# ViktorLiang/GW-Depth

Measured on AMD Instinct MI355X. Metric: images/sec (train fwd+bwd) 480x640 bs=8/GPU, higher is better.
Workload: dtype bf16; 1 GPU; GW-Depth full model (res50 + DETR 6+6 + 4-scale ReferTransformer + decoder) fwd+17 losses+bwd+clip+AdamW, 480x640, bs=8/GPU, dropout 0.1; global_batch=8, parallelism=dp1, launch=hipgraph, graph_segments=1, grad_buckets=8

## Files before the change

### gw_depth_amd/hip.py

```python
import ctypes
import os

import torch

_HERE = os.path.dirname(os.path.abspath(__file__))
LIB_PATH = os.environ.get("GWD_LIB") or os.path.join(_HERE, "libgwdepth_hip.so")

F32, BF16 = 0, 1
ACT_NONE, ACT_RELU, ACT_GELU, ACT_ELU, ACT_SIGMOID = 0, 1, 2, 3, 4
WS_INORM_GELU, WS_RESAMPLE_BWD, WS_EVAL, WS_PLANE, WS_HEALTH, WS_REGIONS, WS_FUSION = 0, 1, 2, 3, 4, 5, 6
GATHER_CONV, GATHER_TRANSPOSED, GATHER_UPSAMPLED = 0, 1, 2
RESAMPLE_BILINEAR_AC, RESAMPLE_NEAREST = 0, 1

ENTRY_POINTS = [
    "gwd_version", "gwd_arch", "gwd_conv_forward", "gwd_conv_wgrad", "gwd_weight_prep", "gwd_act_backward",
    "gwd_colsum", "gwd_layernorm_forward", "gwd_layernorm_backward", "gwd_softmax_forward",
    "gwd_softmax_backward", "gwd_silog_sums", "gwd_silog_backward", "gwd_seg_ce_sum", "gwd_seg_ce_backward",
    "gwd_sqnorm", "gwd_adamw_step", "gwd_resample_forward", "gwd_resample_backward", "gwd_avgpool_forward",
    "gwd_avgpool_backward", "gwd_winattn_forward", "gwd_winattn_backward", "gwd_tokattn_forward",
    "gwd_tokattn_backward", "gwd_tokattn_pair_forward", "gwd_tokattn_pair_backward", "gwd_upsample_taps_collapse", "gwd_upsample_taps_fold", "gwd_certain_sample", "gwd_lsap", "gwd_window_map", "gwd_window_map_multi",
    "gwd_inorm_gelu_forward", "gwd_inorm_gelu_backward", "gwd_weight_prep_batch",
    "gwd_point_sample_forward", "gwd_point_sample_backward", "gwd_act_backward_colsum", "gwd_resample_backward_sep",
    "gwd_softmax_masked_forward", "gwd_softmax_scaled_backward", "gwd_query_workspace", "gwd_eval_accumulate", "gwd_colsum_batch", "gwd_conv_wgrad_batch",
    "gwd_conv_wgrad_takes_bias",
    "gwd_plane_loss_forward", "gwd_plane_loss_backward", "gwd_collate",
    "gwd_anchor_depth_forward", "gwd_anchor_depth_backward", "gwd_mha_flash_forward", "gwd_mha_flash_backward",
    "gwd_ref_scores_forward", "gwd_ref_scores_backward", "gwd_ref_mix_forward", "gwd_ref_mix_backward", "gwd_unpad_add_batch", "gwd_stem_pack", "gwd_stem_forward", "gwd_pos_sine", "gwd_silog_finalize", "gwd_psp_pool_forward", "gwd_psp_pool_backward",
    "gwd_match_cost", "gwd_set_losses_forward", "gwd_set_losses_backward", "gwd_set_losses_focal_forward", "gwd_set_losses_focal_backward", "gwd_resample_u8_pass", "gwd_gather2d", "gwd_point_sample_backward_gather", "gwd_point_sample_framed_forward", "gwd_point_sample_framed_backward", "gwd_stride_place", "gwd_color_adjust", "gwd_bmm",
    "gwd_dense_postprocess", "gwd_line_postprocess", "gwd_line_score",
    "gwd_dense_postprocess_resized",
    "gwd_resample_u8_pass_batch", "gwd_gather2d_batch", "gwd_color_adjust_batch",
    "gwd_pyr_tail_forward", "gwd_pyr_tail_backward", "gwd_pyr_tail_fold_wgrad",
    "gwd_widen_u16_batch",
    "gwd_line_nms",
    "gwd_eval_frames",
    "gwd_segment_stats", "gwd_health_decide", "gwd_adamw_step_guarded",
    "gwd_adamw_step_ema", "gwd_ema_swap",
    "gwd_glass_regions", "gwd_region_planes", "gwd_depth_planar",
    "gwd_line_profiles",
    "gwd_fusion_ring", "gwd_fusion_planes", "gwd_fusion_depth",
    "gwd_render_frames",
]


class HipUnavailable(RuntimeError):
    pass


class ConvDesc(ctypes.Structure):
    _fields_ = [("x", ctypes.c_void_p), ("w", ctypes.c_void_p), ("y", ctypes.c_void_p), ("z", ctypes.c_void_p),
                ("scale", ctypes.c_void_p), ("shift", ctypes.c_void_p), ("residual", ctypes.c_void_p),
                ("zero_page", ctypes.c_void_p), ("mult", ctypes.c_void_p), ("gate", ctypes.c_void_p)] + \
               [(n, ctypes.c_int32) for n in ("B", "Hi", "Wi", "Cin", "Ho", "Wo", "Cout", "KH", "KW", "stride", "pad",
                                              "gather", "Hv", "Wv", "act")] + \
               [("act_scale", ctypes.c_float), ("dtype", ctypes.c_int32), ("gate_act", ctypes.c_int32),
                ("ln_mean", ctypes.c_void_p), ("ln_rstd", ctypes.c_void_p), ("ln_C", ctypes.c_int32), ("reserved", ctypes.c_int32),
                ("dbias", ctypes.c_void_p)]


class BmmDesc(ctypes.Structure):
    _fields_ = [("a", ctypes.c_void_p), ("b", ctypes.c_void_p), ("c", ctypes.c_void_p)] + \
               [(n, ctypes.c_int64) for n in ("a_sb0", "a_sb1", "a_ld", "b_sb0", "b_sb1", "b_ld", "c_sb0", "c_sb1", "c_ld")] + \
               [(n, ctypes.c_int32) for n in ("M", "N", "K", "nb0", "nb1", "a_kmajor", "b_kmajor", "c_is_f32_accumulate", "splits")] + \
               [("alpha", ctypes.c_float), ("dtype", ctypes.c_int32)]


class PrepJob(ctypes.Structure):
    _fields_ = [("w", ctypes.c_void_p), ("row_scale", ctypes.c_void_p), ("w_fwd", ctypes.c_void_p), ("w_dgrad", ctypes.c_void_p),
                ("N", ctypes.c_int32), ("taps", ctypes.c_int32), ("C", ctypes.c_int32), ("block0", ctypes.c_int32),
                ("Np", ctypes.c_int32), ("Cg", ctypes.c_int32), ("Cgp", ctypes.c_int32), ("reserved", ctypes.c_int32)]


class UnpadJob(ctypes.Structure):
    _fields_ = [("src", ctypes.c_void_p), ("dst", ctypes.c_void_p), ("N", ctypes.c_int32), ("taps", ctypes.c_int32), ("G", ctypes.c_int32),
                ("Cg", ctypes.c_int32), ("Cgp", ctypes.c_int32), ("block0", ctypes.c_int32)]


# ... 100 lines not shown


def _zero_page(device):
    if device.type != "cuda":
        return None
    z = _ZERO_PAGES.get(device)
    if z is None:
        z = _ZERO_PAGES[device] = torch.zeros(256, dtype=torch.uint8, device=device)
    return ctypes.c_void_p(z.data_ptr())


def dtype_code(t):
    if t.dtype == torch.float32:
        return F32
    if t.dtype == torch.bfloat16:
        return BF16
    raise TypeError("gw_depth_amd kernels take float32 or bfloat16, got %s" % t.dtype)


def _ptr_pitched(t):
    return None if t is None else ctypes.c_void_p(t.data_ptr())


def _ptr(t):
    if t is None:
        return None
    if not t.is_contiguous():
        raise ValueError("kernel operand must be contiguous")
    return ctypes.c_void_p(t.data_ptr())


class HipLibrary:

    def __init__(self, path=LIB_PATH):
        if not os.path.exists(path):
            raise HipUnavailable(
                "libgwdepth_hip.so not built (%s); run `python -c 'import __graft_entry__ as g; g.build()'`" % path)
        self.lib = ctypes.CDLL(path)
        for name in ENTRY_POINTS:
            if not hasattr(self.lib, name):
                raise HipUnavailable("libgwdepth_hip.so lacks symbol " + name)
        self.lib.gwd_arch.restype = ctypes.c_char_p
        for name in ENTRY_POINTS[2:]:
            getattr(self.lib, name).restype = ctypes.c_int
        L = self.lib
        vp, i32, i64, f32 = ctypes.c_void_p, ctypes.c_int32, ctypes.c_int64, ctypes.c_float
        L.gwd_conv_forward.argtypes = [ctypes.POINTER(ConvDesc), vp]
        L.gwd_conv_wgrad.argtypes = [ctypes.POINTER(ConvDesc), vp, vp]
        L.gwd_weight_prep.argtypes = [vp, vp, vp, vp, i32, i32, i32, i32, vp]
        L.gwd_act_backward.argtypes = [vp, vp, vp, vp, i64, i32, i32, f32, i32, vp]
        L.gwd_colsum.argtypes = [vp, vp, i64, i32, i32, vp]
        L.gwd_conv_wgrad_batch.argtypes = [ctypes.POINTER(ConvDesc), ctypes.POINTER(ctypes.c_void_p), i32, vp]
        L.gwd_conv_wgrad_takes_bias.argtypes = [ctypes.POINTER(ConvDesc), i32]
        L.gwd_plane_loss_forward.argtypes = [vp, vp, vp, vp, i32, i32, i32, i32, vp, vp, vp, i32, vp]
        L.gwd_plane_loss_backward.argtypes = [vp, vp, vp, vp, i32, i32, i32, vp, vp, vp, i32, vp]
        L.gwd_collate.argtypes = [ctypes.POINTER(ImageJob), i32, i32, i32, ctypes.POINTER(ctypes.c_float),
                                  ctypes.POINTER(ctypes.c_float), vp, vp, vp, vp, i32, vp]
        L.gwd_mha_flash_forward.argtypes = [vp, vp, vp, i64, i64, i64, vp, vp, vp, i64, vp, i32, i32, i32, i32, f32, i32, vp]
        L.gwd_mha_flash_backward.argtypes = [vp] * 5 + [i64] * 5 + [vp] * 7 + [i64] * 3 + [i32, i32, i32, i32, f32, i32, vp]
        L.gwd_anchor_depth_forward.argtypes = [vp, vp, vp, i32, i64, i32, i32, vp]
        L.gwd_anchor_depth_backward.argtypes = [vp, vp, vp, vp, vp, i32, i64, i32, i32, vp]
        L.gwd_colsum_batch.argtypes = [ctypes.POINTER(ColsumJob), i32, i32, vp]
        L.gwd_layernorm_forward.argtypes = [vp, vp, vp, vp, vp, vp, vp, i64, i32, i32, i32, i32, vp]
        L.gwd_layernorm_backward.argtypes = [vp, vp, vp, vp, vp, vp, vp, vp, vp, i64, i32, i32, i32, vp, i32, vp]
        L.gwd_unpad_add_batch.argtypes = [ctypes.POINTER(UnpadJob), i32, vp]
        L.gwd_silog_finalize.argtypes = [vp, f32, f32, vp, vp]
        L.gwd_resample_u8_pass.argtypes = [vp, vp, vp, vp, i32, i32, i32, i32, i32, i64, i32, i32, i32, i32, vp]
        L.gwd_gather2d.argtypes = [vp, vp, vp, vp, i32, i32, i64, i32, vp]
        L.gwd_resample_u8_pass_batch.argtypes = [ctypes.POINTER(ResampleJob), i32, i32, i32, vp, i64, vp]
        L.gwd_gather2d_batch.argtypes = [ctypes.POINTER(GatherJob), i32, vp, i64, vp]
        L.gwd_color_adjust_batch.argtypes = [ctypes.POINTER(ColorJob), i32, vp, i32, vp]
        L.gwd_match_cost.argtypes = [vp] * 5 + [i32] * 6 + [f32, f32, vp]
        L.gwd_set_losses_forward.argtypes = [vp] * 9 + [f32] + [vp] * 4 + [i32] * 6 + [vp]
        L.gwd_set_losses_backward.argtypes = [vp] * 8 + [f32] + [vp] * 6 + [i32] * 6 + [vp]
        L.gwd_set_losses_focal_forward.argtypes = [vp] * 9 + [f32] * 2 + [vp] * 4 + [i32] * 6 + [vp]
        L.gwd_set_losses_focal_backward.argtypes = [vp] * 8 + [f32] * 2 + [vp] * 6 + [i32] * 6 + [vp]
        L.gwd_color_adjust.argtypes = [vp, vp, vp, i64, i32, f32, vp]
        L.gwd_bmm.argtypes = [ctypes.POINTER(BmmDesc), vp]
        L.gwd_stride_place.argtypes = [vp, vp, vp] + [i32] * 8 + [vp]
        L.gwd_psp_pool_forward.argtypes = [vp] * 5 + [i32] * 5 + [vp]
        L.gwd_psp_pool_backward.argtypes = [vp] * 6 + [i32] * 6 + [vp]
        L.gwd_pos_sine.argtypes = [vp, vp, vp, vp, vp, i32, i32, i32, i32, i32, i32, i32, vp]
        L.gwd_stem_pack.argtypes = [vp, vp, vp, vp]
        L.gwd_stem_forward.argtypes = [vp, vp, vp, vp, i32, i32, i32, i32, vp]
        L.gwd_softmax_forward.argtypes = [vp, vp, i64, i32, i32, vp]
        L.gwd_softmax_backward.argtypes = [vp, vp, vp, i64, i32, i32, vp]
        L.gwd_silog_sums.argtypes = [vp, vp, vp, i32, i32, i32, i32, i32, i32, i32, vp]
        L.gwd_silog_backward.argtypes = [vp, vp, vp, vp, f32, f32, vp, i32, i32, i32, i32, i32, i32, i32, vp]
        L.gwd_seg_ce_sum.argtypes = [vp, vp, vp, i64, i32, vp]
        L.gwd_seg_ce_backward.argtypes = [vp, vp, vp, f32, vp, i64, i32, vp]
        L.gwd_resample_forward.argtypes = [vp, vp] + [i32] * 9 + [vp]
        L.gwd_resample_backward.argtypes = [vp, vp] + [i32] * 7 + [vp, i32, i32, vp]
        L.gwd_avgpool_forward.argtypes = [vp, vp] + [i32] * 6 + [vp]
        L.gwd_avgpool_backward.argtypes = [vp, vp] + [i32] * 6 + [vp]
        sp = ctypes.POINTER(Strided)
        L.gwd_winattn_forward.argtypes = [sp, sp, sp, sp, vp, vp, i32, vp, i64, i32, i32, i32, f32, i32, vp]
        L.gwd_winattn_backward.argtypes = [sp] * 7 + [vp, vp, vp, i32, vp, i64, i32, i32, i32, f32, i32, i32, vp]
        L.gwd_ref_scores_forward.argtypes = [sp, vp, vp, i32, i32, i32, i32, i32, f32, i32, vp]
        L.gwd_ref_scores_backward.argtypes = [sp, vp, vp, sp, vp, i32, i32, i32, i32, i32, f32, i32, vp]
        L.gwd_ref_mix_forward.argtypes = [vp, vp, vp, vp, i32, i32, i32, i32, i32, i32, vp]
        L.gwd_ref_mix_backward.argtypes = [vp, vp, vp, vp, vp, i32, i32, i32, i32, i32, i32, vp]
        L.gwd_tokattn_forward.argtypes = [sp] * 4 + [i64, i32, i32, f32, i32, vp]
        L.gwd_tokattn_backward.argtypes = [sp] * 7 + [i64, i32, i32, f32, i32, vp]
        L.gwd_upsample_taps_collapse.argtypes = [vp, vp, i32, i32, i32, vp]
        L.gwd_upsample_taps_fold.argtypes = [vp, vp, i32, i32, vp]
        L.gwd_tokattn_pair_forward.argtypes = [sp] * 6 + [i64, i32, i32, f32, i32, vp]
# ... 65 lines not shown
        if n < 0:
            raise ValueError("gwd_query_workspace(%d, %r) -> %d" % (op, dims, n))
        return n

    def version(self):
        return self.lib.gwd_version()

    @staticmethod
    def _desc(x, w, y, dims, z=None, scale=None, shift=None, residual=None, stride=1, pad=0,
              gather=GATHER_CONV, virt=(0, 0), act=ACT_NONE, act_scale=1.0, mult=None, gate=None, gate_act=ACT_NONE, ln=None,
              zero_page=True, dbias=None):
        B, Hi, Wi, Cin, Ho, Wo, Cout, KH, KW = dims
        d = ConvDesc()
        d.x, d.w, d.y, d.z = _ptr(x), _ptr(w), _ptr(y), _ptr(z)
        d.scale, d.shift, d.residual = _ptr(scale), _ptr(shift), _ptr(residual)
        d.zero_page = _zero_page(x.device) if zero_page else None
        d.mult = _ptr(mult)
        d.gate, d.gate_act = _ptr(gate), (gate_act if gate is not None else ACT_NONE)
        d.B, d.Hi, d.Wi, d.Cin, d.Ho, d.Wo, d.Cout, d.KH, d.KW = B, Hi, Wi, Cin, Ho, Wo, Cout, KH, KW
        d.stride, d.pad, d.gather, d.Hv, d.Wv = stride, pad, gather, virt[0], virt[1]
        d.act, d.act_scale, d.dtype = act, act_scale, dtype_code(x)
        if ln is not None:
            d.ln_mean, d.ln_rstd, d.ln_C = _ptr(ln[0]), _ptr(ln[1]), int(ln[2])
        d.dbias = _ptr(dbias)
        return d

    def conv_forward(self, x, w, y, dims, **kw):
        d = self._desc(x, w, y, dims, **kw)
        rc = self.lib.gwd_conv_forward(ctypes.byref(d), self._stream(x, w, y))
        if rc == -4 and kw.get("ln") is not None:
            return False
        if rc == -4 and kw.get("gate") is not None and kw.get("gate_act") == ACT_GELU:
            return False
        self._check(rc, "gwd_conv_forward")

    def conv_wgrad(self, x, gy, dw, dims, **kw):
        d = self._desc(x, None, gy, dims, **kw)
        self._check(self.lib.gwd_conv_wgrad(ctypes.byref(d), _ptr(dw), self._stream(x, gy, dw, kw.get("dbias"))), "gwd_conv_wgrad")

    def conv_wgrad_takes_bias(self, x, gy, dims, batched, **kw):
        d = self._desc(x, None, gy, dims, **kw)
        return self.lib.gwd_conv_wgrad_takes_bias(ctypes.byref(d), 1 if batched else 0) == 1

    def conv_wgrad_batch(self, jobs):
        descs = (ConvDesc * len(jobs))()
        dws = (ctypes.c_void_p * len(jobs))()
        ts = []
        for i, (x, gy, dw, dims, kw) in enumerate(jobs):
            descs[i] = self._desc(x, None, gy, dims, **kw)
            dws[i] = _ptr(dw)
            ts += [x, gy, dw, kw.get("dbias")]
        self._check(self.lib.gwd_conv_wgrad_batch(descs, dws, len(jobs), self._stream(*ts)), "gwd_conv_wgrad_batch")

    def weight_prep(self, w, row_scale, w_fwd, w_dgrad, N, taps, C, dtype):
        self._check(self.lib.gwd_weight_prep(_ptr(w), _ptr(row_scale), _ptr(w_fwd), _ptr(w_dgrad), N, taps, C, dtype,
                                             self._stream(w, w_fwd, w_dgrad)), "gwd_weight_prep")

    def act_backward(self, gy, ref, gx, scale, rows, C, act, act_scale):
        self._check(self.lib.gwd_act_backward(_ptr(gy), _ptr(ref), _ptr(gx), _ptr(scale), rows, C, act, act_scale,
                                              dtype_code(gy), self._stream(gy, ref, gx)), "gwd_act_backward")

    def act_backward_colsum(self, gy, ref, gx, dbias, rows, C, act, act_scale, mult=None):
        rc = self.lib.gwd_act_backward_colsum(_ptr(gy), _ptr(ref), _ptr(gx), _ptr(dbias), rows, C, act, act_scale, _ptr(mult),
                                              dtype_code(gy), self._stream(gy, ref, gx))
        if rc == -4:
            return False
        self._check(rc, "gwd_act_backward_colsum")
        return True

    def colsum(self, g, out, rows, C):
        self._check(self.lib.gwd_colsum(_ptr(g), _ptr(out), rows, C, dtype_code(g), self._stream(g, out)), "gwd_colsum")

    def colsum_batch(self, jobs):
        recs = (ColsumJob * len(jobs))()
        for r, (g, out, rows, C) in zip(recs, jobs):
            r.g, r.out, r.rows, r.C = g.data_ptr(), out.data_ptr(), rows, C
            if not (g.is_contiguous() and out.is_contiguous()):
                raise ValueError("kernel operand must be contiguous")
        ts = [t for j in jobs for t in j[:2]]
        self._check(self.lib.gwd_colsum_batch(recs, len(jobs), dtype_code(jobs[0][0]), self._stream(*ts)), "gwd_colsum_batch")

    @staticmethod
    def colsum_batchable(g, C):
        vec = 8 if g.dtype == torch.bfloat16 else 4
        return C % vec == 0 and C // vec <= 256

    def layernorm_forward(self, x, gamma, beta, y, mean, rstd, rows, C, gelu, residual=None, ld=0):
        self._check(self.lib.gwd_layernorm_forward(_ptr(x), _ptr(gamma), _ptr(beta), _ptr(residual), _ptr(y), _ptr(mean), _ptr(rstd),
                                                   rows, C, ld, int(gelu), dtype_code(x), self._stream(x, y)),
                    "gwd_layernorm_forward")

    def layernorm_backward(self, gy, x, gamma, beta, mean, rstd, gx, dgamma, dbeta, rows, C, gelu, ld=0, gskip=None, elu_input=False):
        flags = int(bool(gelu)) | (2 if elu_input else 0)
        rc = self.lib.gwd_layernorm_backward(_ptr(gy), _ptr(x), _ptr(gamma), _ptr(beta), _ptr(mean), _ptr(rstd), _ptr(gx), _ptr(dgamma),
                                             _ptr(dbeta), rows, C, ld, flags, _ptr(gskip), dtype_code(x), self._stream(gy, x, gx))
        if rc == -4 and (gskip is not None or elu_input):
            self._check(self.lib.gwd_layernorm_backward(_ptr(gy), _ptr(x), _ptr(gamma), _ptr(beta), _ptr(mean), _ptr(rstd), _ptr(gx), _ptr(dgamma),
                                                        _ptr(dbeta), rows, C, ld, int(bool(gelu)), None, dtype_code(x), self._stream(gy, x, gx)),
                        "gwd_layernorm_backward")
            return False
        self._check(rc, "gwd_layernorm_backward")
        return True

    def pos_counts(self, mask_full, mask_level, counts):
        B, H, W = mask_full.shape
        _, h, w = mask_level.shape
# ... 924 lines not shown
```

### gw_depth_amd/model.py

```python
import math
import os

import torch
import torch.nn.functional as F
from torch import nn

from . import ops
from .layers import Conv, FrozenBN, LayerNorm, Linear, Mlp, MlpNorm, Seq
from .ops import ACT_ELU, ACT_GELU, ACT_NONE, ACT_RELU, ACT_SIGMOID

WS = 7
HEADS = 16
DEFAULT_FP32_STAGES = ()


class NestedTensor:

    def __init__(self, tensors, mask):
        self.tensors, self.mask = tensors, mask

    def to(self, device):
        return NestedTensor(self.tensors.to(device), None if self.mask is None else self.mask.to(device))

    def decompose(self):
# ... 753 lines not shown
    def __init__(self, cin, cout):
        super().__init__()
        self.conv = Conv(cin, cout, 3)

    def forward(self, x, size, defer=False, in_gate=ACT_NONE):
        return ops.conv2d(x, self.conv.weight, pad=1, act=ACT_ELU, upsample_to=size, defer=defer, in_gate=in_gate)


class DensePrediction(nn.Module):

    def __init__(self, max_depth, tdim, feat=64):
        super().__init__()
        self.max_depth = max_depth
        self.depth_token_fuse = Mlp(feat + 1 + tdim, None, tdim)
        self.seg_token_fuse = Mlp(feat + tdim, None, tdim)
        for tag in ("depth", "seg"):
            setattr(self, f"upconv1_{tag}", UpConv(tdim, tdim))
            setattr(self, f"norm_{tag}", LayerNorm(tdim))
            setattr(self, f"conv1_{tag}", Seq(_0=Conv(tdim, tdim, 3)))
            setattr(self, f"upconv2_{tag}", UpConv(tdim, tdim // 2))
            setattr(self, f"conv2_{tag}", Seq(_0=Conv(tdim // 2, tdim // 2, 3)))
            if tag == "depth":
                self.get_depth = Seq(_0=Conv(tdim // 2, 1, 3))
        self.get_seg = Conv(tdim // 2, 2, 3)

    def fuse_padded(self, x):
        fc1, fc2 = self.depth_token_fuse.fc1, self.depth_token_fuse.fc2
        pad = x.shape[-1] - fc1.weight.shape[-1]
        if pad == 0:
            return self.depth_token_fuse(x)
        w1 = ops.derived_weight(fc1.weight, pad, lambda: F.pad(fc1.weight, (0, pad, 0, pad)))
        w2 = ops.derived_weight(fc2.weight, pad, lambda: F.pad(fc2.weight, (0, pad)))
        h = ops.linear(x, w1, F.pad(fc1.bias, (0, pad)), ACT_GELU)
        return ops.linear(h, w2, fc2.bias)

    _ZERO_BLOCKS = {}

    @classmethod
    def zero_channels(cls, like, n):
        key = (tuple(like.shape[:3]), n, like.dtype, str(like.device))
        z = cls._ZERO_BLOCKS.get(key)
        if z is None:
            z = cls._ZERO_BLOCKS[key] = torch.zeros(tuple(like.shape[:3]) + (n,), dtype=like.dtype, device=like.device)
        return z

    def branch(self, fuse_in, tag, fuse, size, cast):
        B, H, W, _ = fuse_in.shape
        f = fuse(cast("decoder_fuse", fuse_in))
        f = cast("decoder_up1", f)
        u1 = getattr(self, f"norm_{tag}")(getattr(self, f"upconv1_{tag}")(f, (2 * H, 2 * W), defer=True), in_gate=ACT_ELU)
        c1 = ops.conv2d(u1, getattr(self, f"conv1_{tag}")[0].weight, pad=1, act=ACT_ELU, defer=True)
        c1 = cast("decoder_up2", c1)
        u2 = getattr(self, f"upconv2_{tag}")(c1, size, defer=True, in_gate=ACT_ELU)
        return cast("decoder_head", ops.conv2d(u2, getattr(self, f"conv2_{tag}")[0].weight, pad=1, act=ACT_ELU, in_gate=ACT_ELU))

    def forward(self, feat, depth3, dtok, stok, size, cast=None):
        cast = cast or (lambda stage, t: t)
        B, H, W, _ = feat.shape
        d3 = depth3.view(B, H, W, 1).to(feat.dtype)
        parts = [feat, d3, dtok]
        pad = (-sum(p.shape[-1] for p in parts)) % 32
        if pad and feat.is_cuda:
            parts.append(self.zero_channels(feat, pad))
        d = self.branch(torch.cat(parts, dim=-1), "depth", self.fuse_padded, size, cast)
        depth = ops.conv2d(d, self.get_depth[0].weight, pad=1, act=ACT_SIGMOID, act_scale=float(self.max_depth))
        s = self.branch(torch.cat([feat, stok], dim=-1), "seg", self.seg_token_fuse, size, cast)
        seg = ops.conv2d(s, self.get_seg.weight, pad=1)
        return depth.float().view(B, 1, size[0], size[1]), seg.permute(0, 3, 1, 2)


class GlassRGBD(nn.Module):

    def __init__(self, cfg):
        super().__init__()
        self.cfg = cfg
        self.num_queries = cfg.num_queries
        self.transformer = Transformer(cfg.hidden_dim, cfg.nheads, cfg.enc_layers, cfg.dec_layers,
                                       cfg.dim_feedforward, cfg.dropout)
        self.class_embed = Linear(cfg.hidden_dim, 2)
        self.query_embed = nn.Embedding(cfg.num_queries, cfg.hidden_dim)
        self.input_proj = Conv(2048, cfg.hidden_dim, 1, bias=True)
        self.lines_embed = MLP(cfg.hidden_dim, cfg.hidden_dim, 6, 3)
        self.backbone = Joiner(cfg.hidden_dim, cfg.lr_backbone > 0)
        self.aux_loss = cfg.aux_loss
        self.dense_input_proj = Conv(2048, 512, 1, bias=True)
        self.dense_encoder = ReferTransformer(cfg)
        self.depth_decoder = DensePrediction(cfg.max_depth, cfg.class_token_dim)
        self.compute_dtype = torch.float32
        self.fp32_stages = set(DEFAULT_FP32_STAGES)

    def stage_cast(self, stage, *ts):
        dt = torch.float32 if stage in self.fp32_stages else self.compute_dtype
        out = tuple(t if t.dtype == dt else t.to(dt) for t in ts)
        return out if len(out) > 1 else out[0]

    def decoder_cast(self, stage, t):
        dt = torch.float32 if (stage in self.fp32_stages or "decoder" in self.fp32_stages) else self.compute_dtype
        return t if t.dtype == dt else t.to(dt)

    def forward(self, samples, reflc_points=None, reflc_mat=None, img_name=None, taps=None, match=None):
        if isinstance(samples, (list, torch.Tensor)):
            samples = nested_tensor_from_tensor_list(samples)
        images, pad_mask = samples.decompose()
        H, W = images.shape[-2:]
        cast = self.stage_cast
        x = cast("backbone", to_pixel_major(images))
        feats, masks = self.backbone(x, pad_mask)
        src, mask = feats[3], masks[3]
        pos = pos_sine(mask, self.cfg.hidden_dim // 2, True)
        src_d = cast("detr", src)
        hs = self.transformer(ops.conv2d(src_d, self.input_proj.weight, self.input_proj.bias), mask,
                              self.query_embed.weight, pos)
        logits = self.class_embed(hs).float()
        lines = torch.sigmoid(self.lines_embed(hs).float())
        out = {"pred_logits": logits[-1], "pred_lines": lines[-1]}
        if self.aux_loss:
            out["aux_outputs"] = [{"pred_logits": a, "pred_lines": b} for a, b in zip(logits[:-1], lines[:-1])]
        if match is not None:
            matcher, targets = match
            out["_match_prefetch"] = matcher.prefetch([out] + out.get("aux_outputs", []), targets)
# ... 11 lines not shown
```

### gw_depth_amd/ops.py

```python
import bisect
import os

import torch
import torch.nn.functional as F

from . import hip
from .hip import (ACT_ELU, ACT_GELU, ACT_NONE, ACT_RELU, ACT_SIGMOID, GATHER_CONV, GATHER_TRANSPOSED,
                  GATHER_UPSAMPLED)

__all__ = ["conv2d", "linear", "layer_norm", "softmax_lastdim", "silog_loss", "seg_cross_entropy",
           "ACT_NONE", "ACT_RELU", "ACT_GELU", "ACT_ELU", "ACT_SIGMOID"]


def _lib():
    return hip.library()


class WeightCache:

    def __init__(self, persistent=(), frozen=False):
        self.frozen = bool(frozen)
        self._derived = {}
        self.ranges = sorted((int(a), int(b)) for a, b in persistent)
        self._starts, self._ends, self._merged_from = [], [], -1
# ... 454 lines not shown
        if defer and (act not in (ACT_RELU, ACT_ELU, ACT_GELU) or act_scale != 1.0 or mult is not None or (act == ACT_GELU and fanout)):
            raise ValueError("conv2d: defer needs ReLU / ELU / GELU with act_scale 1 and no dropout multiplier")
        if in_gate not in (ACT_NONE, ACT_RELU, ACT_ELU, ACT_GELU) or (in_gate == ACT_GELU) != (gate_src is not None):
            raise ValueError("conv2d: in_gate is ReLU or ELU, or GELU with the producer's pre-activation tensor as gate_src")
        B, Hi, Wi, Cin = x.shape
        Cout, KH, KW, Cw = w.shape
        if Cw != Cin:
            raise ValueError("conv2d: weight expects %d input channels, input has %d" % (Cw, Cin))
        if virt is None:
            Ho = (Hi + 2 * pad - KH) // stride + 1
            Wo = (Wi + 2 * pad - KW) // stride + 1
            gather, vv = GATHER_CONV, (0, 0)
        else:
            Ho, Wo = virt[0] + 2 * pad - KH + 1, virt[1] + 2 * pad - KW + 1
            gather, vv = GATHER_UPSAMPLED, tuple(virt)
        x = x.contiguous()
        wk = _weight_for(w, row_scale, x.dtype, shadow)
        shift = shift_const if bias is None else (bias.detach().float() if shift_const is None else shift_const + bias.detach().float())
        y = torch.empty((B, Ho, Wo, Cout), dtype=x.dtype, device=x.device)
        need_grad = any(ctx.needs_input_grad[:4])
        z = torch.empty_like(y) if (act == ACT_GELU and need_grad) else None
        if residual is not None:
            residual = residual.contiguous()
        dims = (B, Hi, Wi, Cin, Ho, Wo, Cout, KH, KW)
        if mult is not None:
            mult = mult.contiguous()
        lib.conv_forward(x, wk, y, dims, z=z, shift=shift, residual=residual, stride=stride, pad=pad, gather=gather,
                         virt=vv, act=act, act_scale=act_scale, mult=mult)
        ctx.cfg = (dims, stride, pad, act, act_scale, gather, vv, bias is not None, residual is not None)
        ctx.sinks = sinks
        if mult is not None and (act not in (ACT_NONE, ACT_RELU) or (act == ACT_RELU and residual is not None)):
            raise ValueError("conv2d: a dropout multiplier is supported behind no activation (+ skip) or behind ReLU (no skip) only")
        ctx.save_for_backward(x, w, row_scale, z if act == ACT_GELU else (y if act != ACT_NONE else None), mult, gate_src)
        if defer and act == ACT_GELU:
            if z is None:
                z = y
            ctx.mark_non_differentiable(z)
            ctx.set_materialize_grads(False)
            return y, z
        if fanout:
            return y, x.view_as(x)
        return y

    @staticmethod
    def backward(ctx, gy, *g_fan):
        if gy is None:
            return (None,) * 18
        g_in = _fan_in(ctx, g_fan)
        x, w, row_scale, ref, mult, gate_src = ctx.saved_tensors
        dims, stride, pad, act, act_scale, gather, vv, has_bias, has_res = ctx.cfg
        gy = gy.contiguous()
        w_sink, b_sink = ctx.sinks if ctx.sinks is not None else (None, None)
        want_b = has_bias and ctx.needs_input_grad[2]
        dv, bias_done = _conv_act_backward(gy, ref, mult, act, act_scale, ctx.defer, b_sink if want_b else None, dims)
        gx = g_in
        if ctx.needs_input_grad[0]:
            gx = _conv_dgrad(x, w, row_scale, dv, g_in, dims, stride, pad, gather, vv, ctx.in_gate, gate_src)
        gw, gb = _conv_param_grads(x, w, row_scale, dv, dims, stride, pad, gather, vv, ctx.needs_input_grad[1], want_b and not bias_done,
                                   w_sink, b_sink)
        gres = (gy if mult is not None else dv) if (has_res and ctx.needs_input_grad[3]) else None
        return gx, gw, gb, gres, None, None, None, None, None, None, None, None, None, None, None, None, None, None


def _conv_act_backward(gy, ref, mult, act, act_scale, defer, b_sink, dims):
    lib = _lib()
    rows, Cout = dims[0] * dims[4] * dims[5], dims[6]

    def with_colsum(g, dv, m):
        done = lib.act_backward_colsum(g, ref, dv, b_sink[0], rows, Cout, act, act_scale, mult=m)
        if done and b_sink[1] is not None:
            b_sink[1]()
        return done

    if defer:
        return gy, False
    if mult is not None:
        if b_sink is not None:
            dv = torch.empty_like(gy)
            if with_colsum(gy, dv, mult):
                return dv, True
        gy = gy * mult
    if act == ACT_NONE and act_scale == 1.0:
        return gy, False
    dv = torch.empty_like(gy)
    bias_done = b_sink is not None and with_colsum(gy, dv, None)
    if not bias_done:
        lib.act_backward(gy, ref, dv, None, rows, Cout, act, act_scale)
    return dv, bias_done


def _conv_dgrad(x, w, row_scale, dv, g_in, dims, stride, pad, gather, vv, in_gate, gate_src):
    lib = _lib()
    B, Hi, Wi, Cin, Ho, Wo, Cout, KH, KW = dims
    wt = _weight_transposed(w, row_scale, x.dtype)
    gate = dict(gate=(x if gate_src is None else gate_src), gate_act=in_gate) if in_gate != ACT_NONE else {}
    if (gather == GATHER_UPSAMPLED and x.is_cuda and x.dtype == torch.bfloat16 and KH == 3 and KW == 3
            and pad == 1 and vv == (2 * Hi, 2 * Wi) and row_scale is None and (g_in is None or not gate)):
        gx = torch.empty_like(x)
        lib.conv_forward(dv, _upsampled_dgrad_weight(w, x.dtype), gx, (B, Ho, Wo, Cout, Hi, Wi, Cin, 4, 4), stride=2, pad=1,
                         residual=g_in, **gate)
        return gx
    if gather == GATHER_UPSAMPLED:
        gxv = torch.empty((B, vv[0], vv[1], Cin), dtype=x.dtype, device=x.device)
        lib.conv_forward(dv, wt, gxv, (B, Ho, Wo, Cout, vv[0], vv[1], Cin, KH, KW), stride=1, pad=pad, gather=GATHER_TRANSPOSED)
        if gate and g_in is None:
            return _nearest_upsample_backward(gxv, Hi, Wi, gate=x, gate_act=in_gate)
        gx = _nearest_upsample_backward(gxv, Hi, Wi)
        if g_in is not None:
            gx = gx + g_in
        if gate:
            gated = torch.empty_like(gx)
            lib.act_backward(gx, x, gated, None, B * Hi * Wi, Cin, in_gate, 1.0)
            gx = gated
        return gx
# ... 527 lines not shown
def _pyramid_cat_forward(x, ys):
    lib = _lib()
    x = x.contiguous()
    B, H, W, C = x.shape
    n = len(ys)
    out = torch.empty((B, H, W, (n + 1) * C), dtype=x.dtype, device=x.device)
    out[..., :C].copy_(x)
    shapes = []
    for k, y in enumerate(ys):
        y = y.contiguous()
        if y.shape[0] != B or y.shape[3] != C:
            raise ValueError("pyramid_concat: branch %d has shape %r" % (k, tuple(y.shape)))
        lib.resample_forward(y, out[..., (k + 1) * C:(k + 2) * C], B, y.shape[1], y.shape[2], H, W, C, hip.RESAMPLE_BILINEAR_AC)
        shapes.append((y.shape[1], y.shape[2]))
    return out, (B, H, W, C, shapes)


def _pyramid_cat_backward(cfg, g):
    lib = _lib()
    B, H, W, C, shapes = cfg
    g = g.contiguous()
    grads = [g[..., :C]]
    for k, (h, w) in enumerate(shapes):
        gk = g[..., (k + 1) * C:(k + 2) * C]
        gy = torch.empty((B, h, w, C), dtype=g.dtype, device=g.device)
        tmp = torch.empty(lib.workspace_bytes(hip.WS_RESAMPLE_BWD, B, H, w, C) // 4, dtype=torch.float32, device=g.device)
        if not lib.resample_backward_sep(gk, tmp, gy, B, h, w, H, W, C, hip.RESAMPLE_BILINEAR_AC):
            lib.resample_backward(gk.contiguous(), gy, B, h, w, H, W, C, hip.RESAMPLE_BILINEAR_AC)
        grads.append(gy)
    return grads


class _PyramidCatFn(torch.autograd.Function):

    @staticmethod
    def forward(ctx, x, *ys):
        out, ctx.cfg = _pyramid_cat_forward(x, ys)
        return out

    @staticmethod
    def backward(ctx, g):
        return tuple(_pyramid_cat_backward(ctx.cfg, g))


def pyramid_concat(x, ys):
    C = x.shape[-1]
    if C % 8 or not ys:
        return torch.cat([x] + [upsample_bilinear_ac(y, x.shape[1:3]) for y in ys], dim=-1)
    return _PyramidCatFn.apply(x, *ys)


PYRAMID_TAIL_LOWRES = True
PYRAMID_TAIL_NLOW = 3


class _PyramidTailFn(torch.autograd.Function):

    @staticmethod
    def forward(ctx, x, w, gamma, beta, gelu, nlow, w_sink, ln_sinks, *ys):
        lib = _lib()
        B, H, W, C2 = x.shape
        N = w.shape[0]
        nbr = len(ys)
        if tuple(w.shape) != (N, 3, 3, (1 + nbr) * C2) or not 1 <= nlow <= nbr:
            raise ValueError("pyramid_tail: weight %r does not fit %d branches of %d channels" % (tuple(w.shape), nbr, C2))
        dt = x.dtype
        lows = [y.contiguous() for y in ys[:nlow]]
        cat, cat_cfg = _pyramid_cat_forward(x, ys[nlow:]) if nlow < nbr else (x.contiguous(), None)
        Chi = cat.shape[-1]
        w_hi = derived_weight(w, ("pyr_tail_hi", nlow), lambda: torch.cat([w.detach()[..., :C2], w.detach()[..., (1 + nlow) * C2:]], dim=-1))
        w_lo = [derived_weight(w, ("pyr_tail_lo", k), lambda k=k: w.detach()[..., (k + 1) * C2:(k + 2) * C2].permute(1, 2, 0, 3)
                               .reshape(9 * N, 1, 1, C2).contiguous()) for k in range(nlow)]
        part = torch.empty((B, H, W, N), dtype=dt, device=x.device)
        dims = (B, H, W, Chi, H, W, N, 3, 3)
        lib.conv_forward(cat, _weight_for(w_hi, None, dt), part, dims, stride=1, pad=1)
        Zs = []
        for y, wl in zip(lows, w_lo):
            h, wd = y.shape[1], y.shape[2]
            Z = torch.empty((B, h, wd, 9, N), dtype=dt, device=x.device)
            lib.conv_forward(y, _weight_for(wl, None, dt), Z.view(B, h, wd, 9 * N), (B, h, wd, C2, h, wd, 9 * N, 1, 1), stride=1, pad=0)
            Zs.append(Z)
        need_grad = any(ctx.needs_input_grad)
        out = torch.empty_like(part)
        z = torch.empty_like(part) if need_grad else None
        mean = torch.empty(B * H * W, dtype=torch.float32, device=x.device)
        rstd = torch.empty(B * H * W, dtype=torch.float32, device=x.device)
        g, b = gamma.detach(), beta.detach()
        if lib.pyr_tail_forward(part, Zs, g, b, z, out, mean, rstd, gelu) is False:
            raise ValueError("pyramid_tail: no kernel for N = %d with branches %r" % (N, [tuple(y.shape[1:3]) for y in lows]))
        if need_grad:
            ctx.save_for_backward(cat, w, z, g, b, mean, rstd, *lows)
        ctx.cfg = (dims, bool(gelu), nlow, nbr, C2, w_sink, ln_sinks, cat_cfg, w_hi, w_lo)
        return out

    @staticmethod
    def backward(ctx, gy):
        lib = _lib()
        cat, w, z, g, b, mean, rstd, *lows = ctx.saved_tensors
        dims, gelu, nlow, nbr, C2, w_sink, ln_sinks, cat_cfg, w_hi, w_lo = ctx.cfg
        B, H, W, Chi, _, _, N, _, _ = dims
        dt = cat.dtype
        gz, dg, db = _ln_backward(gy.contiguous(), z, g, b, mean, rstd, gelu, ln_sinks)
        g_cat = _dgrad_stride1(gz, _weight_transposed(w_hi, None, dt), cat, dims, 1)
        g_high = _pyramid_cat_backward(cat_cfg, g_cat) if nlow < nbr else [g_cat]
        Gs = [torch.empty((B, y.shape[1], y.shape[2], 9, N), dtype=dt, device=z.device) for y in lows]
        lib.pyr_tail_backward(gz, Gs)
# ... 856 lines not shown
```

### include/gwdepth.h

```cpp
#ifndef GWDEPTH_H
#define GWDEPTH_H
#include <stdint.h>

#ifdef __cplusplus
extern "C" {
#endif

#define GWD_VERSION 10

enum { GWD_F32 = 0, GWD_BF16 = 1 };
enum { GWD_ACT_NONE = 0, GWD_ACT_RELU = 1, GWD_ACT_GELU = 2, GWD_ACT_ELU = 3, GWD_ACT_SIGMOID = 4 };
enum {
    GWD_GATHER_CONV = 0,
    GWD_GATHER_TRANSPOSED = 1,
    GWD_GATHER_UPSAMPLED = 2
};

typedef struct {
    const void *x;
    const void *w;
    void *y;
    void *z;
    const float *scale;
    const float *shift;
    const void *residual;
    const void *zero_page;
    const void *mult;
    const void *gate;
    int32_t B, Hi, Wi, Cin, Ho, Wo, Cout, KH, KW, stride, pad;
    int32_t gather;
    int32_t Hv, Wv;
    int32_t act;
    float act_scale;
    int32_t dtype;
    int32_t gate_act;
    float *ln_mean;
    float *ln_rstd;
    int32_t ln_C;
    int32_t reserved;
    float *dbias;
} gwd_conv_desc;

int gwd_version(void);
const char *gwd_arch(void);

enum { GWD_WS_INORM_GELU = 0, GWD_WS_RESAMPLE_BWD = 1, GWD_WS_EVAL = 2, GWD_WS_PLANE = 3, GWD_WS_HEALTH = 4, GWD_WS_REGIONS = 5,
       GWD_WS_FUSION = 6 };
int64_t gwd_query_workspace(int32_t op, const int64_t *dims, int32_t ndims);

int gwd_conv_forward(const gwd_conv_desc *d, void *stream);

int gwd_conv_wgrad(const gwd_conv_desc *d, float *dw, void *stream);
int gwd_conv_wgrad_batch(const gwd_conv_desc *descs, float *const *dws, int32_t n, void *stream);
int gwd_conv_wgrad_takes_bias(const gwd_conv_desc *d, int32_t batched);

int gwd_weight_prep(const float *w, const float *row_scale, void *w_fwd, void *w_dgrad, int32_t N,
                    int32_t taps, int32_t C, int32_t dtype, void *stream);

int gwd_act_backward(const void *gy, const void *ref, void *gx, const float *scale, int64_t rows,
                     int32_t C, int32_t act, float act_scale, int32_t dtype, void *stream);

int gwd_colsum(const void *g, float *out, int64_t rows, int32_t C, int32_t dtype, void *stream);
#define GWD_COLSUM_BATCH 16
typedef struct {
    const void *g;
    float *out;
    int64_t rows;
    int32_t C;
    int32_t block0, blocks;
} gwd_colsum_job;
int gwd_colsum_batch(const gwd_colsum_job *jobs, int32_t n_jobs, int32_t dtype, void *stream);
int gwd_act_backward_colsum(const void *gy, const void *ref, void *gx, float *dbias, int64_t rows, int32_t C, int32_t act,
                            float act_scale, const void *mult, int32_t dtype, void *stream);


int gwd_layernorm_forward(const void *x, const float *gamma, const float *beta, const void *residual, void *y, float *mean,
                          float *rstd, int64_t rows, int32_t C, int32_t ld, int32_t gelu, int32_t dtype, void *stream);
#define GWD_LN_ELU_INPUT 2
int gwd_layernorm_backward(const void *gy, const void *x, const float *gamma, const float *beta,
                           const float *mean, const float *rstd, void *gx, float *dgamma, float *dbeta,
                           int64_t rows, int32_t C, int32_t ld, int32_t gelu, const void *gskip, int32_t dtype, void *stream);

int gwd_softmax_forward(const void *x, void *y, int64_t rows, int32_t L, int32_t dtype, void *stream);
int gwd_softmax_backward(const void *gy, const void *y, void *gx, int64_t rows, int32_t L, int32_t dtype,
                         void *stream);
int gwd_softmax_masked_forward(const void *x, const uint8_t *key_mask, void *y, int64_t rows, int32_t L, int64_t rows_per_mask,
                               float scale, int32_t dtype, void *stream);
int gwd_softmax_scaled_backward(const void *gy, const void *y, void *gx, int64_t rows, int32_t L, float scale, int32_t dtype,
                                void *stream);


int gwd_silog_sums(const void *pred, const float *gt, double *sums, int32_t B, int32_t h, int32_t w,
                   int32_t H, int32_t W, int32_t log_depth_error, int32_t dtype, void *stream);
int gwd_silog_finalize(const double *sums, float lambda, float scale, float *loss, void *stream);
int gwd_silog_backward(const void *pred, const float *gt, const double *sums, const float *gloss,
                       float loss_weight, float lambda, void *gpred, int32_t B, int32_t h, int32_t w,
                       int32_t H, int32_t W, int32_t log_depth_error, int32_t dtype, void *stream);

int gwd_seg_ce_sum(const void *logits, const int64_t *target, double *sum, int64_t P, int32_t dtype,
                   void *stream);
int gwd_seg_ce_backward(const void *logits, const int64_t *target, const float *gloss, float scale,
                        void *glogits, int64_t P, int32_t dtype, void *stream);

int gwd_anchor_depth_forward(const void *att, const float *anchor, float *pred, int32_t B, int64_t P, int32_t R,
                             int32_t dtype, void *stream);
int gwd_anchor_depth_backward(const void *att, const float *anchor, const float *gpred, void *datt, float *danchor,
                              int32_t B, int64_t P, int32_t R, int32_t dtype, void *stream);
// ... 400 lines not shown
```

Baseline: 264.8 images/s.

## Fuse thin 3x3 head conv backward (dgrad+wgrad+activation) into one kernel

Adds a dedicated HIP kernel for the backward pass of the final 3x3 convs that map 32 channels to 1 or 2 outputs (depth and seg heads). It computes the sigmoid output-gradient, the input gradient, the ELU gate derivative and the weight gradient in one tiled pass over LDS-staged input, instead of separate act-backward, dgrad and wgrad launches that go through the generic GEMM path. To make this possible, the decoder's last ELU conv is deferred so that the head conv receives the ELU as an input gate. The trade-off is per-block atomic accumulation of the weight gradient and a new specialized code path, with a fallback that applies the gate separately when the kernel declines.

```diff
diff --git a/gw_depth_amd/csrc/thinhead.hip b/gw_depth_amd/csrc/thinhead.hip
--- /dev/null
+++ b/gw_depth_amd/csrc/thinhead.hip
@@ -0,0 +1,194 @@
+#include "common.h"
+
+namespace {
+
+constexpr int C = 32, TILE = 16, HALO = TILE + 2, PIX = 80;
+
+template <int CW> struct Raw;
+template <> struct Raw<8> { typedef uint4 T; };
+template <> struct Raw<4> { typedef uint2 T; };
+
+__device__ __forceinline__ float row_sum16(float v) {
+    v += __builtin_bit_cast(float, __builtin_amdgcn_update_dpp(0, __builtin_bit_cast(int, v), 0xB1, 0xf, 0xf, true));
+    v += __builtin_bit_cast(float, __builtin_amdgcn_update_dpp(0, __builtin_bit_cast(int, v), 0x4E, 0xf, 0xf, true));
+    v += __builtin_bit_cast(float, __builtin_amdgcn_update_dpp(0, __builtin_bit_cast(int, v), 0x141, 0xf, 0xf, true));
+    v += __builtin_bit_cast(float, __builtin_amdgcn_update_dpp(0, __builtin_bit_cast(int, v), 0x140, 0xf, 0xf, true));
+    return v;
+}
+
+template <int NO, bool ELU>
+__global__ __launch_bounds__(256 * NO, 4) void thin_head_bwd_kernel(const __bf16 *__restrict__ x, const __bf16 *__restrict__ gy,
+                                                                    const __bf16 *__restrict__ out_ref, float out_scale,
+                                                                    const uint32_t *__restrict__ wq, __bf16 *__restrict__ dv,
+                                                                    float *__restrict__ dw, int H, int W, int n_tiles) {
+    constexpr int CW = 8 / NO, NT = 256 * NO;
+    __shared__ __attribute__((aligned(16))) char xs[TILE * TILE * PIX];
+    __shared__ float gs[HALO * HALO * NO];
+    const int tw = (W + TILE - 1) / TILE, th = (H + TILE - 1) / TILE;
+    const int lane = threadIdx.x & 63;
+    const int c0 = __builtin_amdgcn_readfirstlane(threadIdx.x >> 6) * CW;
+    float wf[9][NO][CW];
+#pragma unroll
+    for (int tap = 0; tap < 9; ++tap)
+#pragma unroll
+        for (int n = 0; n < NO; ++n)
+#pragma unroll
+            for (int j = 0; j < CW; j += 2) {
+                const uint32_t u = wq[((n * 9 + tap) * C + c0 + j) / 2];
+                wf[tap][n][j] = __builtin_bit_cast(float, u << 16);
+                wf[tap][n][j + 1] = __builtin_bit_cast(float, u & 0xffff0000u);
+            }
+    float wacc[9][NO][CW];
+#pragma unroll
+    for (int tap = 0; tap < 9; ++tap)
+#pragma unroll
+        for (int n = 0; n < NO; ++n)
+#pragma unroll
+            for (int j = 0; j < CW; ++j) wacc[tap][n][j] = 0.f;
+
+    for (int tile = blockIdx.x; tile < n_tiles; tile += gridDim.x) {
+        int t = tile;
+        const int w0 = (t % tw) * TILE;
+        t /= tw;
+        const int h0 = (t % th) * TILE, b = t / th;
+        int tid = threadIdx.x;
+        asm volatile("" : "+v"(tid));
+        constexpr int GK = (HALO * HALO + NT - 1) / NT;
+        __bf16 gv[GK][NO], rv[GK][NO];
+        bool gok[GK];
+#pragma unroll
+        for (int k = 0; k < GK; ++k) {
+            const int i = tid + k * NT, py = i / HALO, px = i - py * HALO;
+            const int ih = h0 + py - 1, iw = w0 + px - 1;
+            gok[k] = i < HALO * HALO && (unsigned)ih < (unsigned)H && (unsigned)iw < (unsigned)W;
+            const size_t o = (((size_t)b * H + (gok[k] ? ih : h0)) * W + (gok[k] ? iw : w0)) * NO;
+#pragma unroll
+            for (int n = 0; n < NO; ++n) {
+                gv[k][n] = gy[o + n];
+                if (out_ref) rv[k][n] = out_ref[o + n];
+            }
+        }
+        uint4 val[TILE * TILE * 4 / NT];
+#pragma unroll
+        for (int k = 0; k < TILE * TILE * 4 / NT; ++k) {
+            const int i = tid + k * NT, v = i & 3, p = i >> 2;
+            const int ih = h0 + (p >> 4), iw = w0 + (p & 15);
+            const bool ok = ih < H && iw < W;
+            val[k] = *(const uint4 *)(x + (((size_t)b * H + (ok ? ih : h0)) * W + (ok ? iw : w0)) * C + v * 8);
+            if (!ok) val[k] = make_uint4(0u, 0u, 0u, 0u);
+        }
+#pragma unroll
+        for (int k = 0; k < GK; ++k) {
+            const int i = tid + k * NT;
+#pragma unroll
+            for (int n = 0; n < NO; ++n) {
+                float g = (float)gv[k][n];
+                if (out_ref) {
+                    const float sg = (float)rv[k][n] / out_scale;
+                    g *= sg * (1.0f - sg);
+                    g *= out_scale;
+                    g = (float)(__bf16)g;
+                }
+                if (i < HALO * HALO) gs[i * NO + n] = gok[k] ? g : 0.f;
+            }
+        }
+#pragma unroll
+        for (int k = 0; k < TILE * TILE * 4 / NT; ++k) {
+            const int i = tid + k * NT;
+            *(uint4 *)(xs + (i >> 2) * PIX + (i & 3) * 16) = val[k];
+        }
+        __syncthreads();
+#pragma unroll 1
+        for (int p = lane; p < TILE * TILE; p += 64) {
+            const int ty = p >> 4, tx = p & 15;
+            float g[9][NO];
+#pragma unroll
+            for (int kh = 0; kh < 3; ++kh)
+#pragma unroll
+                for (int kw = 0; kw < 3; ++kw)
+#pragma unroll
+                    for (int n = 0; n < NO; ++n) g[kh * 3 + kw][n] = gs[((ty + 2 - kh) * HALO + tx + 2 - kw) * NO + n];
+            char *slot = xs + p * PIX + c0 * 2;
+            const typename Raw<CW>::T raw = *(const typename Raw<CW>::T *)slot;
+            const __bf16 *xb = (const __bf16 *)&raw;
+            float xf[CW], acc[CW];
+#pragma unroll
+            for (int j = 0; j < CW; ++j) {
+                xf[j] = (float)xb[j];
+                acc[j] = 0.f;
+            }
+#pragma unroll
+            for (int tap = 0; tap < 9; ++tap)
+#pragma unroll
+                for (int n = 0; n < NO; ++n)
+#pragma unroll
+                    for (int j = 0; j < CW; ++j) {
+                        acc[j] = __builtin_fmaf(g[tap][n], wf[tap][n][j], acc[j]);
+                        wacc[tap][n][j] = __builtin_fmaf(g[tap][n], xf[j], wacc[tap][n][j]);
+                    }
+            typename Raw<CW>::T outraw;
+            __bf16 *ob = (__bf16 *)&outraw;
+#pragma unroll
+            for (int j = 0; j < CW; ++j) {
+                float o = (float)(__bf16)acc[j];
+                if (ELU) o *= (xf[j] > 0.f ? 1.0f : xf[j] + 1.0f);
+                ob[j] = (__bf16)o;
+            }
+            *(typename Raw<CW>::T *)slot = outraw;
+        }
+        __syncthreads();
+        for (int i = tid; i < TILE * TILE * 4; i += NT) {
+            const int v = i & 3, p = i >> 2;
+            const int ih = h0 + (p >> 4), iw = w0 + (p & 15);
+            if (ih < H && iw < W) *(uint4 *)(dv + (((size_t)b * H + ih) * W + iw) * C + v * 8) = *(const uint4 *)(xs + p * PIX + v * 16);
+        }
+    }
+    float *red = (float *)xs;
+    __syncthreads();
+#pragma unroll
+    for (int tap = 0; tap < 9; ++tap)
+#pragma unroll
+        for (int n = 0; n < NO; ++n)
+#pragma unroll
+            for (int j = 0; j < CW; ++j) {
+                float s = row_sum16(wacc[tap][n][j]);
+                s += __shfl_xor(s, 16);
+                s += __shfl_xor(s, 32);
+                if (lane == 0) red[(n * 9 + tap) * C + c0 + j] = s;
+            }
+    __syncthreads();
+    for (int i = threadIdx.x; i < 9 * NO * C; i += NT) unsafeAtomicAdd(dw + i, red[i]);
+}
+
+template <int NO>
+void launch(bool elu, int grid, hipStream_t s, const void *x, const void *gy, const void *out_ref, float out_scale, const void *w, void *dv,
+            float *dw, int H, int W, int tiles) {
+    if (elu)
+        thin_head_bwd_kernel<NO, true><<<grid, 256 * NO, 0, s>>>((const __bf16 *)x, (const __bf16 *)gy, (const __bf16 *)out_ref, out_scale,
+                                                                 (const uint32_t *)w, (__bf16 *)dv, dw, H, W, tiles);
+    else
+        thin_head_bwd_kernel<NO, false><<<grid, 256 * NO, 0, s>>>((const __bf16 *)x, (const __bf16 *)gy, (const __bf16 *)out_ref, out_scale,
+                                                                  (const uint32_t *)w, (__bf16 *)dv, dw, H, W, tiles);
+}
+
+}
+
+extern "C" int gwd_thin_head_backward(const void *x, const void *gy, const void *w, void *dv, float *dw, int32_t B, int32_t H, int32_t W,
+                                      int32_t Cin, int32_t Cout, int32_t k, int32_t stride, int32_t pad, int32_t gate_act,
+                                      const void *out_ref, int32_t out_act, float out_act_scale, int32_t dtype, void *stream) {
+    if (!x || !gy || !w || !dv || !dw || B < 0 || H <= 0 || W <= 0) return -1;
+    if (dtype != GWD_BF16 || Cin != C || (Cout != 1 && Cout != 2) || k != 3 || stride != 1 || pad != 1) return 0;
+    if (gate_act != GWD_ACT_NONE && gate_act != GWD_ACT_ELU) return 0;
+    if (out_ref ? (out_act != GWD_ACT_SIGMOID || !(out_act_scale > 0.f)) : out_act != GWD_ACT_NONE) return 0;
+    if (((uintptr_t)x | (uintptr_t)dv | (uintptr_t)w) & 15 || ((uintptr_t)gy | (uintptr_t)out_ref) & 1 || (uintptr_t)dw & 3) return 0;
+    const int64_t tiles = (int64_t)B * ((H + TILE - 1) / TILE) * ((W + TILE - 1) / TILE);
+    if (tiles >= (1LL << 31)) return 0;
+    if (tiles == 0) return 1;
+    const int cap = 1024 / Cout;
+    const int grid = (int)(tiles < cap ? tiles : cap);
+    hipStream_t s = (hipStream_t)stream;
+    if (Cout == 1) launch<1>(gate_act == GWD_ACT_ELU, grid, s, x, gy, out_ref, out_act_scale, w, dv, dw, H, W, (int)tiles);
+    else launch<2>(gate_act == GWD_ACT_ELU, grid, s, x, gy, out_ref, out_act_scale, w, dv, dw, H, W, (int)tiles);
+    GWD_CHECK_LAUNCH();
+    return 1;
+}
diff --git a/gw_depth_amd/hip.py b/gw_depth_amd/hip.py
--- a/gw_depth_amd/hip.py
+++ b/gw_depth_amd/hip.py
@@ -22,7 +22,7 @@
     "gwd_inorm_gelu_forward", "gwd_inorm_gelu_backward", "gwd_weight_prep_batch",
     "gwd_point_sample_forward", "gwd_point_sample_backward", "gwd_act_backward_colsum", "gwd_resample_backward_sep",
     "gwd_softmax_masked_forward", "gwd_softmax_scaled_backward", "gwd_query_workspace", "gwd_eval_accumulate", "gwd_colsum_batch", "gwd_conv_wgrad_batch",
-    "gwd_conv_wgrad_takes_bias",
+    "gwd_conv_wgrad_takes_bias", "gwd_thin_head_backward",
     "gwd_plane_loss_forward", "gwd_plane_loss_backward", "gwd_collate",
     "gwd_anchor_depth_forward", "gwd_anchor_depth_backward", "gwd_mha_flash_forward", "gwd_mha_flash_backward",
     "gwd_ref_scores_forward", "gwd_ref_scores_backward", "gwd_ref_mix_forward", "gwd_ref_mix_backward", "gwd_unpad_add_batch", "gwd_stem_pack", "gwd_stem_forward", "gwd_pos_sine", "gwd_silog_finalize", "gwd_psp_pool_forward", "gwd_psp_pool_backward",
@@ -229,6 +229,7 @@
         L.gwd_colsum.argtypes = [vp, vp, i64, i32, i32, vp]
         L.gwd_conv_wgrad_batch.argtypes = [ctypes.POINTER(ConvDesc), ctypes.POINTER(ctypes.c_void_p), i32, vp]
         L.gwd_conv_wgrad_takes_bias.argtypes = [ctypes.POINTER(ConvDesc), i32]
+        L.gwd_thin_head_backward.argtypes = [vp] * 5 + [i32] * 9 + [vp, i32, f32, i32, vp]
         L.gwd_plane_loss_forward.argtypes = [vp, vp, vp, vp, i32, i32, i32, i32, vp, vp, vp, i32, vp]
         L.gwd_plane_loss_backward.argtypes = [vp, vp, vp, vp, i32, i32, i32, vp, vp, vp, i32, vp]
         L.gwd_collate.argtypes = [ctypes.POINTER(ImageJob), i32, i32, i32, ctypes.POINTER(ctypes.c_float),
@@ -400,6 +401,20 @@
             ts += [x, gy, dw, kw.get("dbias")]
         self._check(self.lib.gwd_conv_wgrad_batch(descs, dws, len(jobs), self._stream(*ts)), "gwd_conv_wgrad_batch")
 
+    def thin_head_backward(self, x, gy, w, dv, dw, dims, stride=1, pad=1, gate_act=ACT_NONE, out_ref=None, out_act=ACT_NONE,
+                           out_act_scale=1.0):
+        B, Hi, Wi, Cin, Ho, Wo, Cout, KH, KW = dims
+        if (Ho, Wo) != (Hi, Wi) or KH != KW or dtype_code(gy) != dtype_code(x) or dtype_code(w) != dtype_code(x) or dv.dtype != x.dtype:
+            return False
+        rc = self.lib.gwd_thin_head_backward(_ptr(x), _ptr(gy), _ptr(w), _ptr(dv), _ptr(dw), B, Hi, Wi, Cin, Cout, KH, stride, pad, gate_act,
+                                             _ptr(out_ref), out_act if out_ref is not None else ACT_NONE, out_act_scale, dtype_code(x),
+                                             self._stream(x, gy, w, dv, dw, out_ref))
+        if rc == 0:
+            return False
+        if rc != 1:
+            self._check(rc, "gwd_thin_head_backward")
+        return True
+
     def weight_prep(self, w, row_scale, w_fwd, w_dgrad, N, taps, C, dtype):
         self._check(self.lib.gwd_weight_prep(_ptr(w), _ptr(row_scale), _ptr(w_fwd), _ptr(w_dgrad), N, taps, C, dtype,
                                              self._stream(w, w_fwd, w_dgrad)), "gwd_weight_prep")
diff --git a/gw_depth_amd/model.py b/gw_depth_amd/model.py
--- a/gw_depth_amd/model.py
+++ b/gw_depth_amd/model.py
@@ -829,7 +829,10 @@
         c1 = ops.conv2d(u1, getattr(self, f"conv1_{tag}")[0].weight, pad=1, act=ACT_ELU, defer=True)
         c1 = cast("decoder_up2", c1)
         u2 = getattr(self, f"upconv2_{tag}")(c1, size, defer=True, in_gate=ACT_ELU)
-        return cast("decoder_head", ops.conv2d(u2, getattr(self, f"conv2_{tag}")[0].weight, pad=1, act=ACT_ELU, in_gate=ACT_ELU))
+        defer = (ops.THIN_HEAD_FUSED and u2.is_cuda and u2.dtype == torch.bfloat16 and torch.is_grad_enabled()
+                 and cast("decoder_head", u2) is u2)
+        c2 = ops.conv2d(u2, getattr(self, f"conv2_{tag}")[0].weight, pad=1, act=ACT_ELU, in_gate=ACT_ELU, defer=defer)
+        return cast("decoder_head", c2), (ACT_ELU if defer else ACT_NONE)
 
     def forward(self, feat, depth3, dtok, stok, size, cast=None):
         cast = cast or (lambda stage, t: t)
@@ -839,10 +842,10 @@
         pad = (-sum(p.shape[-1] for p in parts)) % 32
         if pad and feat.is_cuda:
             parts.append(self.zero_channels(feat, pad))
-        d = self.branch(torch.cat(parts, dim=-1), "depth", self.fuse_padded, size, cast)
-        depth = ops.conv2d(d, self.get_depth[0].weight, pad=1, act=ACT_SIGMOID, act_scale=float(self.max_depth))
-        s = self.branch(torch.cat([feat, stok], dim=-1), "seg", self.seg_token_fuse, size, cast)
-        seg = ops.conv2d(s, self.get_seg.weight, pad=1)
+        d, gate = self.branch(torch.cat(parts, dim=-1), "depth", self.fuse_padded, size, cast)
+        depth = ops.conv2d(d, self.get_depth[0].weight, pad=1, act=ACT_SIGMOID, act_scale=float(self.max_depth), in_gate=gate)
+        s, gate = self.branch(torch.cat([feat, stok], dim=-1), "seg", self.seg_token_fuse, size, cast)
+        seg = ops.conv2d(s, self.get_seg.weight, pad=1, in_gate=gate)
         return depth.float().view(B, 1, size[0], size[1]), seg.permute(0, 3, 1, 2)
 
 
diff --git a/gw_depth_amd/ops.py b/gw_depth_amd/ops.py
--- a/gw_depth_amd/ops.py
+++ b/gw_depth_amd/ops.py
@@ -530,14 +530,50 @@
         gy = gy.contiguous()
         w_sink, b_sink = ctx.sinks if ctx.sinks is not None else (None, None)
         want_b = has_bias and ctx.needs_input_grad[2]
+        in_gate = ctx.in_gate
+        if (THIN_HEAD_FUSED and all(ctx.needs_input_grad[:2]) and g_in is None and not (has_bias or has_res or ctx.defer)
+                and _is_thin_head(x, w, row_scale, mult, gate_src, dims, stride, pad, gather, act, in_gate)):
+            done = _thin_head_backward(x, w, gy, ref, act, act_scale, in_gate, dims, w_sink)
+            if done is not None:
+                return (done[0], done[1]) + (None,) * 16
+            in_gate = ACT_NONE
         dv, bias_done = _conv_act_backward(gy, ref, mult, act, act_scale, ctx.defer, b_sink if want_b else None, dims)
         gx = g_in
         if ctx.needs_input_grad[0]:
-            gx = _conv_dgrad(x, w, row_scale, dv, g_in, dims, stride, pad, gather, vv, ctx.in_gate, gate_src)
+            gx = _conv_dgrad(x, w, row_scale, dv, g_in, dims, stride, pad, gather, vv, in_gate, gate_src)
+            if in_gate != ctx.in_gate:
+                gated = torch.empty_like(gx)
+                _lib().act_backward(gx, x, gated, None, dims[0] * dims[1] * dims[2], dims[3], ctx.in_gate, 1.0)
+                gx = gated
         gw, gb = _conv_param_grads(x, w, row_scale, dv, dims, stride, pad, gather, vv, ctx.needs_input_grad[1], want_b and not bias_done,
                                    w_sink, b_sink)
         gres = (gy if mult is not None else dv) if (has_res and ctx.needs_input_grad[3]) else None
         return gx, gw, gb, gres, None, None, None, None, None, None, None, None, None, None, None, None, None, None
+
+
+def _on_device(t):
+    return t.is_cuda
+
+
+def _is_thin_head(x, w, row_scale, mult, gate_src, dims, stride, pad, gather, act, in_gate):
+    B, Hi, Wi, Cin, Ho, Wo, Cout, KH, KW = dims
+    return (_on_device(x) and x.dtype == torch.bfloat16 and (KH, KW, stride, pad) == (3, 3, 1, 1) and Cin == 32 and Cout in (1, 2)
+            and gather == GATHER_CONV and row_scale is None and mult is None and gate_src is None
+            and in_gate in (ACT_NONE, ACT_ELU) and act in (ACT_NONE, ACT_SIGMOID))
+
+
+def _thin_head_backward(x, w, gy, ref, act, act_scale, in_gate, dims, w_sink):
+    gx = torch.empty_like(x)
+    gw = w_sink[0] if w_sink is not None else torch.zeros(w.shape, dtype=torch.float32, device=w.device)
+    wk = _weight_for(w, None, x.dtype, getattr(w, "_gwd_bf16", None))
+    fold = dict(out_ref=ref, out_act=act, out_act_scale=act_scale) if act != ACT_NONE else {}
+    if _lib().thin_head_backward(x, gy, wk, gx, gw, dims, gate_act=in_gate, **fold) is False:
+        return None
+    if w_sink is None:
+        return gx, gw
+    if w_sink[1] is not None:
+        w_sink[1]()
+    return gx, None
 
 
 def _conv_act_backward(gy, ref, mult, act, act_scale, defer, b_sink, dims):
@@ -1171,6 +1207,7 @@
 
 PYRAMID_TAIL_LOWRES = True
 PYRAMID_TAIL_NLOW = 3
+THIN_HEAD_FUSED = True
 
 
 class _PyramidTailFn(torch.autograd.Function):
diff --git a/include/gwdepth.h b/include/gwdepth.h
--- a/include/gwdepth.h
+++ b/include/gwdepth.h
@@ -53,6 +53,10 @@
 int gwd_conv_wgrad(const gwd_conv_desc *d, float *dw, void *stream);
 int gwd_conv_wgrad_batch(const gwd_conv_desc *descs, float *const *dws, int32_t n, void *stream);
 int gwd_conv_wgrad_takes_bias(const gwd_conv_desc *d, int32_t batched);
+
+int gwd_thin_head_backward(const void *x, const void *gy, const void *w, void *dv, float *dw, int32_t B, int32_t H, int32_t W,
+                           int32_t Cin, int32_t Cout, int32_t k, int32_t stride, int32_t pad, int32_t gate_act,
+                           const void *out_ref, int32_t out_act, float out_act_scale, int32_t dtype, void *stream);
 
 int gwd_weight_prep(const float *w, const float *row_scale, void *w_fwd, void *w_dgrad, int32_t N,
                     int32_t taps, int32_t C, int32_t dtype, void *stream);
```

Result: no change. 267.0 images/s, median of 6 (+0.8%).
